# j-fu/ExtendableSparse.jl

Measured on AMD Instinct MI355X. Metric: assembled+flushed nnz/sec and HBM GB/s %peak, 256³ 7-pt stencil, 1/2/4/8 GPU, higher is better.
Workload: dtype f64; 1 GPU; fdrand 256^3 Float64/Int64 fresh build: device COO append (the producer writes every update to its radix bucket) -> LDS bucket sort + ordered fold -> CSC (BASELINE.json configs[1]); n=256, appended_entries=200933376, final_nnz=117047296, partition=producer-side (append = partition), parallelism=1 GPU

## Files before the change

### extendablesparse.jl_amd/csrc/local_x.hip

```cpp
#include "generators.hpp"
#include "local.hpp"
#include "pair.hpp"

namespace esplocal {

namespace {
constexpr int G_ROWS = 7;
constexpr int G_CAP = THREADS * G_ROWS;
}

struct StencilColumn {
    i64 stride[3];
    bool lo[3], hi[3], b[3];
    double vlo[3], vhi[3], vb[3];
};

template <class F>
__device__ __forceinline__ double draw_if(bool on, F f) {
    return __ballot(on) != 0 ? f() : 0.0;
}

struct FdSource {
    i64 nx, ny, nz;
    double hx, hy, hz;
    u64 seed;
    int rand_mode;
    int fast;
    int div_mid;
    u64 magic_nx, magic_nxny;
    u64 zsub[3];

    struct Consts {
        espgen::SharedDiv x, y, z;
        __device__ __forceinline__ explicit Consts(const FdSource &s) : x(s.hx), y(s.hy), z(s.hz) {}
    };
    __device__ __forceinline__ double over(double n, const espgen::SharedDiv &by) const {
        return div_mid ? by.quot_mid(n) : n / by.d;
    }
    __device__ __forceinline__ u64 z0(i64 g) const { return seed + (6ull * (u64)g + 1ull) * ESP_GOLDEN; }

    __device__ __forceinline__ void upper(const Consts &k, i64 g, StencilColumn &c) const {
        i64 i, j, kk;
        espgen::fd_node(*this, g, &i, &j, &kk);
        const int md = rand_mode;
        const u64 zg = z0(g);
        c.stride[0] = nx * ny, c.stride[1] = nx, c.stride[2] = 1;
        c.lo[0] = kk > 1, c.lo[1] = j > 1, c.lo[2] = i > 1;
        c.hi[0] = i < nx, c.hi[1] = j < ny, c.hi[2] = kk < nz;
        c.b[0] = i == 1 || i == nx;
        c.b[1] = ny > 2 && (j == 1 || j == ny);
        c.b[2] = nz > 2 && (kk == 1 || kk == nz);
        c.vhi[0] = over(espgen::fd_rand_z(md, zg, 0) * hy * hz, k.x);
        c.vhi[1] = over(espgen::fd_rand_z(md, zg, 2) * hx * hz, k.y);
        c.vhi[2] = over(espgen::fd_rand_z(md, zg, 4) * hx * hy, k.z);
    }
    __device__ __forceinline__ void lower(const Consts &k, i64 g, int t, const double *sx, const double *sy, StencilColumn &c) const {
        const int md = rand_mode;
        const u64 zg = z0(g);
        const bool x_in = c.lo[2] && t >= 1, y_in = c.lo[1] && (i64)t >= nx;
        const double x_lds = sx[x_in ? t - 1 : 0], y_lds = sy[y_in ? t - (int)nx : 0];
        c.vlo[0] = draw_if(c.lo[0], [&] { return over(espgen::fd_rand_z(md, zg - zsub[0], 4) * hx * hy, k.z); });
        const double y_drawn = draw_if(c.lo[1] && !y_in, [&] { return over(espgen::fd_rand_z(md, zg - zsub[1], 2) * hx * hz, k.y); });
        const double x_drawn = draw_if(c.lo[2] && !x_in, [&] { return over(espgen::fd_rand_z(md, zg - zsub[2], 0) * hy * hz, k.x); });
        c.vlo[1] = y_in ? y_lds : y_drawn;
        c.vlo[2] = x_in ? x_lds : x_drawn;
        c.vb[0] = draw_if(c.b[0], [&] { return espgen::fd_rand_z(md, zg, 1) * hy * hz; });
        c.vb[1] = draw_if(c.b[1], [&] { return espgen::fd_rand_z(md, zg, 3) * hx * hz; });
        c.vb[2] = draw_if(c.b[2], [&] { return espgen::fd_rand_z(md, zg, 5) * hx * hy; });
    }
};

template <int KEYS, class SRC, bool KEEP>
__global__ __launch_bounds__(THREADS, 6) void pair_gen_pred_k(Args a, SRC src, const u64 *pred, u64 out_cap) {
    static_assert(KEYS == 1 || KEYS == 2, "one kind: 2 = every update is an UPDATE");
    constexpr bool UPD = KEYS == 2;
    __shared__ u32 srow[KEEP ? 1 : G_CAP];
    __shared__ double sval[G_CAP];
    __shared__ double shx[THREADS], shy[THREADS];
    __shared__ u32 lw[WAVES];

    const int t = threadIdx.x, lane = t & 63, w = t >> 6;
    const int s = (int)(a.first + (i64)blockIdx.x);
    if (s >= a.S) return;
    const u64 dst = esp_uniform_u64(pred[s]);
    const u64 dst_next = esp_uniform_u64(pred[s + 1]);
    const int ncl = 2 << a.cl_bits;
    const u64 hi = ((u64)s << (a.rem_bits + 1)) + a.base;
    const i64 c_lo = (i64)(hi >> a.rb);
    const i64 c_hi = min(c_lo + (i64)ncl, a.col_end);
    const bool has = c_lo + t < c_hi;
    bool present[G_ROWS];
    double acc[G_ROWS];
    u32 row[G_ROWS];
#pragma unroll
    for (int q = 0; q < G_ROWS; q++) present[q] = false, acc[q] = 0.0, row[q] = 0u;
    const typename SRC::Consts k(src);
    StencilColumn c;
    if (has) {
        src.upper(k, c_lo + t, c);
        shx[t] = c.vhi[0];
        shy[t] = c.vhi[1];
    }
    __syncthreads();
    if (has) {
        src.lower(k, c_lo + t, t, shx, shy, c);
        const i64 l = c_lo + t + 1;
        auto step = [&](int q, bool on, double v) {
            if (!on) return;
            if constexpr (UPD)
                espfold::fold_step_update(present[q], acc[q], v);
            else
                espfold::fold_step_sel(present[q], acc[q], a.kind32, v);
        };
#pragma unroll
        for (int q = 0; q < 3; q++) {
            row[q] = (u32)(l - c.stride[q]);
            row[4 + q] = (u32)(l + c.stride[2 - q]);
            step(q, c.lo[q], -c.vlo[q]);
        }
        row[3] = (u32)l;
#pragma unroll
        for (int q = 0; q < 3; q++) step(3, c.lo[q], c.vlo[q]);
#pragma unroll
        for (int q = 0; q < 3; q++) {
            step(3, c.hi[q], c.vhi[q]);
            step(3, c.b[q], c.vb[q]);
        }
#pragma unroll
        for (int q = 0; q < 3; q++) step(4 + q, c.hi[q], -c.vhi[q]);
    }
    u32 ec = 0;
#pragma unroll
    for (int q = 0; q < G_ROWS; q++) ec += present[q] ? 1u : 0u;
    const PairPlace pl = pair_place(ec, lw, lane, w);
    if (!pair_table_hit(dst, dst_next, pl.total, out_cap, s)) {
        if (t == 0) a.host_words[1] = (u64)PRED_MISS;
        return;
    }
    {
        u32 at = pl.at0;
#pragma unroll
        for (int q = 0; q < G_ROWS; q++) {
            if (present[q]) {
                if constexpr (!KEEP) srow[at] = row[q];
                sval[at] = acc[q];
                at++;
            }
        }
    }
    __syncthreads();
    pair_store<KEEP>(a, srow, sval, 0, dst, pl, hi, ncl, s, t);
    if (s == a.S - 1 && t == 0) a.host_words[0] = pair_grand_total(dst, pl.total);
}

bool launch_pair_gen_predicted(const Variant &v, unsigned grid, hipStream_t stream, const Args &a, const espgen::FdArgs &fd, const u64 *pred,
                               u64 out_cap, bool keep) {
    if (!v.fresh || v.pieces || a.cl_bits < 0 || (2 << a.cl_bits) > THREADS || a.rb >= 32 || !a.colptr_out || !a.host_words) return false;
    auto mid = [](double h) { return h >= 0x1.0p-100 && h <= 0x1.0p100; };
    const FdSource src{fd.nx, fd.ny, fd.nz, fd.hx, fd.hy, fd.hz, fd.seed, fd.rand_mode, fd.fast, mid(fd.hx) && mid(fd.hy) && mid(fd.hz),
                       fd.magic_nx, fd.magic_nxny,
                       {6ull * (u64)(fd.nx * fd.ny) * ESP_GOLDEN, 6ull * (u64)fd.nx * ESP_GOLDEN, 6ull * ESP_GOLDEN}};
    return pair_for_keys(v.keys, [&](auto K) {
        constexpr int KEYS = decltype(K)::value;
        if (keep)
            hipLaunchKernelGGL((pair_gen_pred_k<KEYS, FdSource, true>), dim3(grid), dim3(THREADS), 0, stream, a, src, pred, out_cap);
        else
            hipLaunchKernelGGL((pair_gen_pred_k<KEYS, FdSource, false>), dim3(grid), dim3(THREADS), 0, stream, a, src, pred, out_cap);
    });
}

}
```

### extendablesparse.jl_amd/csrc/pair.hpp

```cpp
#pragma once
#include <type_traits>

#include "local_args.hpp"

namespace esplocal {

struct PairPlace {
    u32 at0, total;
};
__device__ __forceinline__ PairPlace pair_place(u32 ec, u32 *lw, int lane, int w) {
    const u32 einc = esp_wave_scan_add(ec);
    if (lane == 63) lw[w] = einc;
    __syncthreads();
    PairPlace pl{einc - ec, 0u};
#pragma unroll
    for (int i = 0; i < WAVES; i++) {
        pl.at0 += i < w ? lw[i] : 0u;
        pl.total += lw[i];
    }
    return pl;
}

__device__ __forceinline__ bool pair_table_hit(u64 dst, u64 dst_next, u32 total, u64 out_cap, int s) {
    return dst_next >= dst && dst_next - dst == (u64)total && dst <= out_cap && (u64)total <= out_cap - dst && (s > 0 || dst == 0);
}

template <bool KEEP>
__device__ __forceinline__ void pair_store(const Args &a, const u32 *rows, const double *vals, i64 row_add, u64 dst, PairPlace pl, u64 hi,
                                           int ncl, int s, int t) {
    for (int p = t; p < (int)pl.total; p += THREADS) {
        if constexpr (!KEEP) a.out_row[dst + p] = (i64)rows[p] + row_add;
        a.out_val[dst + p] = vals[p];
    }
    if constexpr (!KEEP) {
        const i64 c_lo = (i64)(hi >> a.rb);
        const i64 c_hi = min(c_lo + (i64)ncl, a.col_end);
        if (c_lo + t < c_hi) a.colptr_out[c_lo + t] = (i64)(dst + pl.at0) + 1;
        if (s == a.S - 1 && t == 0) a.colptr_out[a.col_end] = (i64)(dst + pl.total) + 1;
    }
}

__device__ __forceinline__ u64 pair_grand_total(u64 dst, u32 total) { return ST_PRE | ((dst + (u64)total) & ST_VAL); }

template <class F>
bool pair_for_keys(int keys, F f) {
    if (keys == 1) return f(std::integral_constant<int, 1>{}), true;
    if (keys == 2) return f(std::integral_constant<int, 2>{}), true;
    return false;
}

}
```

Measured before the change: 533.9 billion nnz/s.

## Specialize stencil generator on rand mode, fold diagonal directly, vectorize pair stores

Templates the FD source on the random mode so it is a compile-time constant, and recomputes boundary flags from node indices instead of storing bool arrays. When every update is an UPDATE and values are positive, the per-row fold sequence is replaced by directly setting each row's presence and summing the diagonal. The output store writes 16-byte vector pairs when the row and value arrays share alignment, and the wave index is made uniform with readfirstlane. The launcher now rejects non-mid-range h values instead of falling back to exact division, which shrinks the path's coverage and relies on the positive-mode fold matching the fold semantics.

```diff
diff --git a/extendablesparse.jl_amd/csrc/local_x.hip b/extendablesparse.jl_amd/csrc/local_x.hip
--- a/extendablesparse.jl_amd/csrc/local_x.hip
+++ b/extendablesparse.jl_amd/csrc/local_x.hip
@@ -11,8 +11,13 @@
 
 struct StencilColumn {
     i64 stride[3];
-    bool lo[3], hi[3], b[3];
+    i64 i, j, k, nx, ny, nz;
     double vlo[3], vhi[3], vb[3];
+    __device__ __forceinline__ bool lo(int q) const { return q == 0 ? k > 1 : q == 1 ? j > 1 : i > 1; }
+    __device__ __forceinline__ bool hi(int q) const { return q == 0 ? i < nx : q == 1 ? j < ny : k < nz; }
+    __device__ __forceinline__ bool b(int q) const {
+        return q == 0 ? (i == 1 || i == nx) : q == 1 ? (ny > 2 && (j == 1 || j == ny)) : (nz > 2 && (k == 1 || k == nz));
+    }
 };
 
 template <class F>
@@ -20,13 +25,13 @@
     return __ballot(on) != 0 ? f() : 0.0;
 }
 
+template <int MODE>
 struct FdSource {
+    static constexpr bool positive = MODE == 0 || MODE == 1;
     i64 nx, ny, nz;
     double hx, hy, hz;
     u64 seed;
-    int rand_mode;
     int fast;
-    int div_mid;
     u64 magic_nx, magic_nxny;
     u64 zsub[3];
 
@@ -35,38 +40,33 @@
         __device__ __forceinline__ explicit Consts(const FdSource &s) : x(s.hx), y(s.hy), z(s.hz) {}
     };
     __device__ __forceinline__ double over(double n, const espgen::SharedDiv &by) const {
-        return div_mid ? by.quot_mid(n) : n / by.d;
+        return by.quot_mid(n);
     }
     __device__ __forceinline__ u64 z0(i64 g) const { return seed + (6ull * (u64)g + 1ull) * ESP_GOLDEN; }
 
     __device__ __forceinline__ void upper(const Consts &k, i64 g, StencilColumn &c) const {
-        i64 i, j, kk;
-        espgen::fd_node(*this, g, &i, &j, &kk);
-        const int md = rand_mode;
+        espgen::fd_node(*this, g, &c.i, &c.j, &c.k);
+        constexpr int md = MODE;
         const u64 zg = z0(g);
         c.stride[0] = nx * ny, c.stride[1] = nx, c.stride[2] = 1;
-        c.lo[0] = kk > 1, c.lo[1] = j > 1, c.lo[2] = i > 1;
-        c.hi[0] = i < nx, c.hi[1] = j < ny, c.hi[2] = kk < nz;
-        c.b[0] = i == 1 || i == nx;
-        c.b[1] = ny > 2 && (j == 1 || j == ny);
-        c.b[2] = nz > 2 && (kk == 1 || kk == nz);
+        c.nx = nx, c.ny = ny, c.nz = nz;
         c.vhi[0] = over(espgen::fd_rand_z(md, zg, 0) * hy * hz, k.x);
         c.vhi[1] = over(espgen::fd_rand_z(md, zg, 2) * hx * hz, k.y);
         c.vhi[2] = over(espgen::fd_rand_z(md, zg, 4) * hx * hy, k.z);
     }
     __device__ __forceinline__ void lower(const Consts &k, i64 g, int t, const double *sx, const double *sy, StencilColumn &c) const {
-        const int md = rand_mode;
+        constexpr int md = MODE;
         const u64 zg = z0(g);
-        const bool x_in = c.lo[2] && t >= 1, y_in = c.lo[1] && (i64)t >= nx;
+        const bool x_in = c.lo(2) && t >= 1, y_in = c.lo(1) && (i64)t >= nx;
         const double x_lds = sx[x_in ? t - 1 : 0], y_lds = sy[y_in ? t - (int)nx : 0];
-        c.vlo[0] = draw_if(c.lo[0], [&] { return over(espgen::fd_rand_z(md, zg - zsub[0], 4) * hx * hy, k.z); });
-        const double y_drawn = draw_if(c.lo[1] && !y_in, [&] { return over(espgen::fd_rand_z(md, zg - zsub[1], 2) * hx * hz, k.y); });
-        const double x_drawn = draw_if(c.lo[2] && !x_in, [&] { return over(espgen::fd_rand_z(md, zg - zsub[2], 0) * hy * hz, k.x); });
+        c.vlo[0] = draw_if(c.lo(0), [&] { return over(espgen::fd_rand_z(md, zg - zsub[0], 4) * hx * hy, k.z); });
+        const double y_drawn = draw_if(c.lo(1) && !y_in, [&] { return over(espgen::fd_rand_z(md, zg - zsub[1], 2) * hx * hz, k.y); });
+        const double x_drawn = draw_if(c.lo(2) && !x_in, [&] { return over(espgen::fd_rand_z(md, zg - zsub[2], 0) * hy * hz, k.x); });
         c.vlo[1] = y_in ? y_lds : y_drawn;
         c.vlo[2] = x_in ? x_lds : x_drawn;
-        c.vb[0] = draw_if(c.b[0], [&] { return espgen::fd_rand_z(md, zg, 1) * hy * hz; });
-        c.vb[1] = draw_if(c.b[1], [&] { return espgen::fd_rand_z(md, zg, 3) * hx * hz; });
-        c.vb[2] = draw_if(c.b[2], [&] { return espgen::fd_rand_z(md, zg, 5) * hx * hy; });
+        c.vb[0] = draw_if(c.b(0), [&] { return espgen::fd_rand_z(md, zg, 1) * hy * hz; });
+        c.vb[1] = draw_if(c.b(1), [&] { return espgen::fd_rand_z(md, zg, 3) * hx * hz; });
+        c.vb[2] = draw_if(c.b(2), [&] { return espgen::fd_rand_z(md, zg, 5) * hx * hy; });
     }
 };
 
@@ -74,6 +74,7 @@
 __global__ __launch_bounds__(THREADS, 6) void pair_gen_pred_k(Args a, SRC src, const u64 *pred, u64 out_cap) {
     static_assert(KEYS == 1 || KEYS == 2, "one kind: 2 = every update is an UPDATE");
     constexpr bool UPD = KEYS == 2;
+    constexpr bool FLAGS = UPD && SRC::positive;
     __shared__ u32 srow[KEEP ? 1 : G_CAP];
     __shared__ double sval[G_CAP];
     __shared__ double shx[THREADS], shy[THREADS];
@@ -105,29 +106,46 @@
     if (has) {
         src.lower(k, c_lo + t, t, shx, shy, c);
         const i64 l = c_lo + t + 1;
-        auto step = [&](int q, bool on, double v) {
-            if (!on) return;
-            if constexpr (UPD)
-                espfold::fold_step_update(present[q], acc[q], v);
-            else
-                espfold::fold_step_sel(present[q], acc[q], a.kind32, v);
-        };
 #pragma unroll
-        for (int q = 0; q < 3; q++) {
-            row[q] = (u32)(l - c.stride[q]);
-            row[4 + q] = (u32)(l + c.stride[2 - q]);
-            step(q, c.lo[q], -c.vlo[q]);
+        for (int q = 0; q < 3; q++) row[q] = (u32)(l - c.stride[q]), row[4 + q] = (u32)(l + c.stride[2 - q]);
+        row[3] = (u32)l;
+        if constexpr (FLAGS) {
+#pragma unroll
+            for (int q = 0; q < 3; q++) {
+                present[q] = c.lo(q), acc[q] = -c.vlo[q];
+                present[4 + q] = c.hi(q), acc[4 + q] = -c.vhi[q];
+            }
+            bool any = false;
+            double d = 0.0;
+#pragma unroll
+            for (int q = 0; q < 3; q++) any = any || c.lo(q), d = d + (c.lo(q) ? c.vlo[q] : 0.0);
+#pragma unroll
+            for (int q = 0; q < 3; q++) {
+                any = any || c.hi(q) || c.b(q);
+                d = d + (c.hi(q) ? c.vhi[q] : 0.0);
+                d = d + (c.b(q) ? c.vb[q] : 0.0);
+            }
+            present[3] = any, acc[3] = d;
+        } else {
+            auto step = [&](int q, bool on, double v) {
+                if (!on) return;
+                if constexpr (UPD)
+                    espfold::fold_step_update(present[q], acc[q], v);
+                else
+                    espfold::fold_step_sel(present[q], acc[q], a.kind32, v);
+            };
+#pragma unroll
+            for (int q = 0; q < 3; q++) step(q, c.lo(q), -c.vlo[q]);
+#pragma unroll
+            for (int q = 0; q < 3; q++) step(3, c.lo(q), c.vlo[q]);
+#pragma unroll
+            for (int q = 0; q < 3; q++) {
+                step(3, c.hi(q), c.vhi[q]);
+                step(3, c.b(q), c.vb[q]);
+            }
+#pragma unroll
+            for (int q = 0; q < 3; q++) step(4 + q, c.hi(q), -c.vhi[q]);
         }
-        row[3] = (u32)l;
-#pragma unroll
-        for (int q = 0; q < 3; q++) step(3, c.lo[q], c.vlo[q]);
-#pragma unroll
-        for (int q = 0; q < 3; q++) {
-            step(3, c.hi[q], c.vhi[q]);
-            step(3, c.b[q], c.vb[q]);
-        }
-#pragma unroll
-        for (int q = 0; q < 3; q++) step(4 + q, c.hi[q], -c.vhi[q]);
     }
     u32 ec = 0;
 #pragma unroll
@@ -157,16 +175,22 @@
                                u64 out_cap, bool keep) {
     if (!v.fresh || v.pieces || a.cl_bits < 0 || (2 << a.cl_bits) > THREADS || a.rb >= 32 || !a.colptr_out || !a.host_words) return false;
     auto mid = [](double h) { return h >= 0x1.0p-100 && h <= 0x1.0p100; };
-    const FdSource src{fd.nx, fd.ny, fd.nz, fd.hx, fd.hy, fd.hz, fd.seed, fd.rand_mode, fd.fast, mid(fd.hx) && mid(fd.hy) && mid(fd.hz),
-                       fd.magic_nx, fd.magic_nxny,
-                       {6ull * (u64)(fd.nx * fd.ny) * ESP_GOLDEN, 6ull * (u64)fd.nx * ESP_GOLDEN, 6ull * ESP_GOLDEN}};
-    return pair_for_keys(v.keys, [&](auto K) {
-        constexpr int KEYS = decltype(K)::value;
-        if (keep)
-            hipLaunchKernelGGL((pair_gen_pred_k<KEYS, FdSource, true>), dim3(grid), dim3(THREADS), 0, stream, a, src, pred, out_cap);
-        else
-            hipLaunchKernelGGL((pair_gen_pred_k<KEYS, FdSource, false>), dim3(grid), dim3(THREADS), 0, stream, a, src, pred, out_cap);
-    });
+    if (!(mid(fd.hx) && mid(fd.hy) && mid(fd.hz))) return false;
+    auto go = [&](auto M) {
+        using Src = FdSource<decltype(M)::value>;
+        const Src src{fd.nx, fd.ny, fd.nz, fd.hx, fd.hy, fd.hz, fd.seed, fd.fast, fd.magic_nx, fd.magic_nxny,
+                      {6ull * (u64)(fd.nx * fd.ny) * ESP_GOLDEN, 6ull * (u64)fd.nx * ESP_GOLDEN, 6ull * ESP_GOLDEN}};
+        return pair_for_keys(v.keys, [&](auto K) {
+            constexpr int KEYS = decltype(K)::value;
+            if (keep)
+                hipLaunchKernelGGL((pair_gen_pred_k<KEYS, Src, true>), dim3(grid), dim3(THREADS), 0, stream, a, src, pred, out_cap);
+            else
+                hipLaunchKernelGGL((pair_gen_pred_k<KEYS, Src, false>), dim3(grid), dim3(THREADS), 0, stream, a, src, pred, out_cap);
+        });
+    };
+    if (fd.rand_mode == 0) return go(std::integral_constant<int, 0>{});
+    if (fd.rand_mode == 1) return go(std::integral_constant<int, 1>{});
+    return go(std::integral_constant<int, 2>{});
 }
 
 }
diff --git a/extendablesparse.jl_amd/csrc/pair.hpp b/extendablesparse.jl_amd/csrc/pair.hpp
--- a/extendablesparse.jl_amd/csrc/pair.hpp
+++ b/extendablesparse.jl_amd/csrc/pair.hpp
@@ -13,9 +13,10 @@
     if (lane == 63) lw[w] = einc;
     __syncthreads();
     PairPlace pl{einc - ec, 0u};
+    const int wu = __builtin_amdgcn_readfirstlane(w);
 #pragma unroll
     for (int i = 0; i < WAVES; i++) {
-        pl.at0 += i < w ? lw[i] : 0u;
+        pl.at0 += i < wu ? lw[i] : 0u;
         pl.total += lw[i];
     }
     return pl;
@@ -28,9 +29,37 @@
 template <bool KEEP>
 __device__ __forceinline__ void pair_store(const Args &a, const u32 *rows, const double *vals, i64 row_add, u64 dst, PairPlace pl, u64 hi,
                                            int ncl, int s, int t) {
-    for (int p = t; p < (int)pl.total; p += THREADS) {
-        if constexpr (!KEEP) a.out_row[dst + p] = (i64)rows[p] + row_add;
-        a.out_val[dst + p] = vals[p];
+    typedef double dbl2 __attribute__((ext_vector_type(2)));
+    typedef long long ll2 __attribute__((ext_vector_type(2)));
+    const int total = (int)pl.total;
+    double *const ov = a.out_val + dst;
+    i64 *orow = nullptr;
+    bool wide = true;
+    if constexpr (!KEEP) {
+        orow = a.out_row + dst;
+        wide = (((uintptr_t)ov ^ (uintptr_t)orow) & 8) == 0;
+    }
+    if (wide) {
+        const int head = (int)(((uintptr_t)ov >> 3) & 1);
+        if (t == 0 && head && total > 0) {
+            if constexpr (!KEEP) orow[0] = (i64)rows[0] + row_add;
+            ov[0] = vals[0];
+        }
+        const int npair = (total - head) >> 1;
+        for (int q = t; q < npair; q += THREADS) {
+            const int p = head + 2 * q;
+            if constexpr (!KEEP) *reinterpret_cast<ll2 *>(orow + p) = ll2{(i64)rows[p] + row_add, (i64)rows[p + 1] + row_add};
+            *reinterpret_cast<dbl2 *>(ov + p) = dbl2{vals[p], vals[p + 1]};
+        }
+        if (t == ESP_WAVE && total > head && ((total - head) & 1)) {
+            if constexpr (!KEEP) orow[total - 1] = (i64)rows[total - 1] + row_add;
+            ov[total - 1] = vals[total - 1];
+        }
+    } else {
+        for (int p = t; p < total; p += THREADS) {
+            if constexpr (!KEEP) orow[p] = (i64)rows[p] + row_add;
+            ov[p] = vals[p];
+        }
     }
     if constexpr (!KEEP) {
         const i64 c_lo = (i64)(hi >> a.rb);
```

New measurement: 575.1 billion nnz/s, median of 6. 1.08x the previous value.
